# ChrisTho23/DrakeGPT

Measured on AMD Instinct MI355X. Metric: training tokens/sec (fwd+bwd+AdamW), higher is better.
Workload: dtype bf16; 1 GPU; TransformerLM_scaled: V=80 C=384 T=256 heads=6 layers=6 dropout=0.2; fwd+bwd+AdamW; hipGraph=on; batch_per_gpu=64, global_batch=64, seq_len=256, parallelism=dp1, dp_gradient_buckets=1, params=10800464

## Files before the change

drakegpt_amd/_lib.py:

```python
from __future__ import annotations

import ctypes as C
import os

import torch

_HERE = os.path.dirname(os.path.abspath(__file__))
LIB_PATH = os.path.join(_HERE, "lib", "libdrakegpt_hip.so")

DG_F32 = 0
DG_BF16 = 1
DG_FP8_E4M3 = 2
DG_FP8_E5M2 = 3
DG_F32X3 = 4
ABI_VERSION = 21


class GemmNtArgs(C.Structure):
    _fields_ = [
        ("A", C.c_void_p), ("lda", C.c_int64),
        ("B", C.c_void_p), ("ldb", C.c_int64),
        ("C", C.c_void_p), ("ldc", C.c_int64),
        ("M", C.c_int32), ("N", C.c_int32), ("K", C.c_int32),
        ("in_dtype", C.c_int32), ("out_dtype", C.c_int32),
# ... 88 lines not shown
    "dg_gemm_nt_colsum_rows": [C.POINTER(GemmNtArgs)],
    "dg_gemm_nt_sign_bits_bytes": [_i, _i],
    "dg_fp8_amax": [_vp, _i, _i64, _vp, _i, _vp, _vp],
    "dg_fp8_quantize": [_vp, _i, _vp, _i, _i64, _vp, _i, _vp, _vp, _vp],
    "dg_fp8_quantize_delayed": [_vp, _i, _vp, _i, _i64, _vp, _vp, _vp, _vp],
    "dg_gemm_tn": [_vp, _i64, _vp, _i64, _vp, _i64, _i64, _i, _i, _i, _i, _i, _vp],
    "dg_gemm_tn_grouped": [C.POINTER(TnProblem), _i, _i, _vp, _i64, _vp],
    "dg_gemm_tn_grouped_workspace_bytes": [C.POINTER(TnProblem), _i],
    "dg_reduce_partials": [_vp, _i64, _i, _vp, _i64, _vp],
    "dg_colsum": [_vp, _i64, _i, _vp, _i64, _i, _i, _i, _vp],
    "dg_dropout_bwd_cast": [_vp, _i, _i64, _vp, _i64, _i, _i, _i, _f, _vp, _u32, _vp, _i64, _vp, _i64, _i, _vp],
    "dg_cast": [_vp, _i, _vp, _i, _i64, _vp],
    "dg_transpose_cast": [_vp, _i64, _vp, _i64, _i, _i, _i, _vp],
    "dg_transpose_cast_batched": [_vp, _i, _i, _i, _i, _vp],
    "dg_transpose_u8_batched": [_vp, _i, _i, _vp],
    "dg_attn_keep_bits_bytes": [_i, _i, _i, _i, _i],
    "dg_attn_fwd": [_vp, _vp, _vp, _i, _i, _i, _i, _f, _f, _vp, _u32, _i, _vp, _i64, _vp],
    "dg_attn_bwd": [_vp, _vp, _vp, _vp, _vp, _vp, _i64, _i, _i, _i, _i, _f, _f, _vp, _u32, _i, _vp, _i64, _vp],
    "dg_attn_fp8_out_supported": [_i, _i, _i, _i, _i],
    "dg_attn_fwd_fp8": [_vp, _vp, _vp, _i, _i, _i, _i, _f, _f, _vp, _u32, _i, _vp, _i64, C.POINTER(AttnFp8Out), _vp],
    "dg_attn_bwd_fp8": [_vp, _vp, _vp, _vp, _vp, _vp, _i64, _i, _i, _i, _i, _f, _f, _vp, _u32, _i, _vp, _i64, C.POINTER(AttnFp8Out), _vp],
    "dg_attn_bwd_workspace_bytes": [_i, _i, _i, _i, _i],
    "dg_attn_decode": [_vp, _vp, _i, _i, _i, _i, _i, _f, _i, _vp],
    "dg_attn_decode_append": [_vp, _vp, _vp, _vp, _i, _i, _i, _i, _f, _i, _vp],
    "dg_embed_window": [_vp, _i64, _vp, _vp, _vp, _vp, _i, _i, _i, _i, _i, _vp],
    "dg_sample_rows": [_vp, _i64, _i, _i, _vp, _vp, _vp, _i64, _vp, _i64, _vp],
    "dg_sample_rows_nucleus": [_vp, _i64, _i, _i, _vp, _vp, _vp, _i64, _vp, _i64, _vp],
    "dg_cross_entropy": [_vp, _i, _i64, _vp, _vp, _vp, _i64, _i, _f, _vp, _i, _i, _vp],
    "dg_cross_entropy_fp8": [_vp, _i64, _vp, _vp, _vp, _i64, _f, _i, _i, _vp, _i64, _vp],
    "dg_cross_entropy_fused": [_vp, _i64, _vp, _vp, _vp, _i64, _i, _f, _i, _i, _vp, _i64, _i, _vp, _vp, _vp, _f, _vp],
# ... 1 lines not shown
    "dg_cross_entropy_fp8_smooth": [_vp, _i64, _vp, _vp, _vp, _i64, _f, _i, _i, _vp, _i64, _f, _vp],
    "dg_cross_entropy_fused_smooth": [_vp, _i64, _vp, _vp, _vp, _i64, _i, _f, _i, _i, _vp, _i64, _i, _vp, _vp, _vp, _f, _f, _f, _vp],
    "dg_reduce_sum": [_vp, _i64, _f, _vp, _vp],
    "dg_softmax_rows": [_vp, _i64, _vp, _i64, _i, _i, _vp],
    "dg_adamw_step": [_vp, _vp, _vp, _vp, _i64, _vp, _vp, _f, _vp, _i, _vp],
    "dg_sumsq_parts": [_i64],
    "dg_sumsq_partials": [_vp, _i64, _vp, _vp],
    "dg_grad_norm_finalize": [_vp, _i, _f, _vp, _vp, _vp],
    "dg_adamw_step_clip": [_vp, _vp, _vp, _vp, _i64, _vp, _vp, _f, _vp, _vp, _i, _vp],
    "dg_adamw_step_sched": [_vp, _vp, _vp, _vp, _i64, _vp, _vp, _f, _vp, _vp, _i64, _vp, _vp, _i, _vp],
    "dg_adamw_step_ema": [_vp, _vp, _vp, _vp, _i64, _vp, _vp, _f, _vp, _vp, _i64, _vp, _vp, _i, _vp, _vp, _vp],
    "dg_swap_f32": [_vp, _vp, _i64, _vp],
    "dg_grad_accumulate": [_vp, _vp, _i64, _vp, _vp, _vp, _vp, _vp],
    "dg_block_chain_supported": [_i, _i],
    "dg_block_chain_fwd": [C.POINTER(BlockChainArgs), _vp],
    "dg_l2_warm": [_vp, _i64, _vp],
    "dg_pack_chain_weights": [_vp, _i64, _vp, _i, _i, _vp],
    "dg_pack_chain_weights_batched": [_vp, _i, _i, _vp],
    "dg_block_chain_bwd_supported": [_i, _i],
    "dg_block_chain_bwd": [C.POINTER(BlockChainBwdArgs), _vp],
}


def _load() -> C.CDLL:
    if not os.path.exists(LIB_PATH):
        raise RuntimeError(
            f"drakegpt_amd: {LIB_PATH} is missing. Build it with `python -m drakegpt_amd.build` "
            "(needs hipcc; cross-compiles for gfx950 without a GPU). There is no CPU fallback.")
    lib = C.CDLL(LIB_PATH)
    for name, argtypes in SIGNATURES.items():
# ... 27 lines not shown
```

drakegpt_amd/csrc/chain.hip:

```cpp
#include "common.h"
#include <stdlib.h>

typedef __attribute__((address_space(1))) const void* gptr_t;
typedef __attribute__((address_space(3))) void* lptr_t;

#define CH_C 384
#define CH_ROWS 64
#define CH_STAGE_B 24576
#define CH_STAGE_A 4096
#define CH_STAGE (CH_STAGE_B + CH_STAGE_A)
#define CH_NST 4
#define CH_ARES (CH_NST * CH_STAGE)
#define CH_KS (CH_C / 32)

struct ChainP {
    const char* o;
    const float* x;
    const char* wproj; const float* bproj;
    float* x1;
    const float* ln2w; const float* ln2b; float* mean2; float* rstd2; bf16_t* h2;
    const char* w1; const float* b1; bf16_t* f; unsigned char* bits;
    const char* w2; const float* b2;
    float* x2; bf16_t* x2b;
    const float* ln1w; const float* ln1b; float* mean1; float* rstd1; bf16_t* h1;
    const char* wqkv; bf16_t* qkv;
    int M, n_blocks;
    float eps;
    const uint32_t* rng; uint32_t site_proj, site_ffn, thr; float inv_keep; int drop;
    int stagger;
    unsigned long long* stamps;
    int dbg;
};

__device__ __forceinline__ void ch_wait_vm(int n) {
    switch (n) {
        case 6: asm volatile("s_waitcnt vmcnt(6)" ::: "memory"); break;
        case 7: asm volatile("s_waitcnt vmcnt(7)" ::: "memory"); break;
        case 12: asm volatile("s_waitcnt vmcnt(12)" ::: "memory"); break;
        case 13: asm volatile("s_waitcnt vmcnt(13)" ::: "memory"); break;
        case 14: asm volatile("s_waitcnt vmcnt(14)" ::: "memory"); break;
        case 8: asm volatile("s_waitcnt vmcnt(8)" ::: "memory"); break;
        case 18: asm volatile("s_waitcnt vmcnt(18)" ::: "memory"); break;
        case 20: asm volatile("s_waitcnt vmcnt(20)" ::: "memory"); break;
        default: asm volatile("s_waitcnt vmcnt(0)" ::: "memory"); break;
    }
// ... 264 lines not shown
        if (HAS_QKV) warm(w3, p.wqkv, 3 * KS);
        asm volatile("s_waitcnt vmcnt(0)" : "+v"(w0), "+v"(w1), "+v"(w2), "+v"(w3) :: "memory");
    }
    auto stamp = [&](int k) {
        if (p.stamps && wave == 0) {
            const unsigned long long t = __builtin_amdgcn_s_memtime();
            if (lane == 0) p.stamps[(int64_t)blockIdx.x * 24 + k] = t;
        }
    };
    u32x4 fa0[2], fb0[6], fa1[2], fb1[6];
    for (int blk = blockIdx.x; blk < p.n_blocks; blk += gridDim.x) {
        const int64_t row0 = (int64_t)blk * CH_ROWS;
        int g = 0;
        if (MODE == 2) {
            float xv[2][3][8];
#pragma unroll
            for (int q = 0; q < 3; ++q)
#pragma unroll
                for (int i = 0; i < 2; ++i) {
                    const float* xp = p.x + row0 * C + mad24(wm * 32 + i * 16 + fr, C, col_l + 32 * q);
                    const f32x4 a = *(const f32x4*)xp, b = *(const f32x4*)(xp + 4);
#pragma unroll
                    for (int e = 0; e < 4; ++e) { xv[i][q][e] = a[e]; xv[i][q][4 + e] = b[e]; }
                }
            layernorm(xv, (float*)(lds + 0 * CH_STAGE + CH_STAGE_B), row0, p.ln1w, p.ln1b, p.mean1, p.rstd1, p.h1);
        }
        __builtin_amdgcn_s_barrier();
        auto pipe_barrier = [&]() {
            __builtin_amdgcn_sched_barrier(0);
            asm volatile("s_waitcnt lgkmcnt(0)" ::: "memory");
            __builtin_amdgcn_s_barrier();
            __builtin_amdgcn_sched_barrier(0);
        };
        auto piece = [&](int nstep, bool ring_a, bool next, bool a_after_barrier, bool drain = false) {
            read_B(fb0, g);
            if (!a_after_barrier) { if (ring_a) read_A_ring(fa0, g); else read_A_res(fa0, 0); }
            for (int t = 0; t < nstep; t += 2) {
                if (drain && t == nstep - 2 && p.dbg != 10) asm volatile("s_waitcnt vmcnt(0)" ::: "memory");
                if (t == 8) asm volatile("s_waitcnt vmcnt(0)" ::: "memory");
// ... 169 lines not shown
        int dev = 0, n = 256;
        if (hipGetDevice(&dev) == hipSuccess) {
            int x = 0;
            if (hipDeviceGetAttribute(&x, hipDeviceAttributeMultiprocessorCount, dev) == hipSuccess && x > 0) n = x;
        }
        return n;
    }();
    return v;
}

extern "C" int dg_block_chain_supported(int M, int C) { return M > 0 && M % CH_ROWS == 0 && C == CH_C; }

static unsigned long long* g_chain_stamps = nullptr;
extern "C" void dg_debug_set_chain_fwd_stamps(void* q) { g_chain_stamps = (unsigned long long*)q; }

extern "C" int dg_block_chain_fwd(const dg_block_chain_args* a, void* stream) {
    if (!a || !dg_block_chain_supported(a->M, a->C)) return DG_ERR_ARG;
    if (a->mode < 0 || a->mode > 4) return DG_ERR_ARG;
    if (a->dropout_p < 0.f || a->dropout_p >= 1.f) return DG_ERR_ARG;
    const int m = a->mode;
    const bool has_proj = m == 0 || m == 1 || m == 3, has_ffn1 = m == 0 || m == 1, has_ffn2 = m == 0 || m == 1 || m == 4;
    const bool has_qkv = m == 0 || m == 2, ln1 = m == 0 || m == 2 || m == 4;
    auto al = [](const void* q) { return q && dg_aligned16(q); };
    if (!al(a->x) && m != 4) return DG_ERR_ARG;
    if (has_proj && (!al(a->o) || !al(a->wproj) || !al(a->bproj) || !al(a->x1) || !al(a->ln2w) || !al(a->ln2b) || !a->mean2 || !a->rstd2 || !al(a->h2)))
        return DG_ERR_ARG;
    if (has_ffn1 && (!al(a->w1) || !al(a->b1) || !a->sign_bits ||
                     a->sign_bits_bytes < (int64_t)((a->M + 127) / 128) * (4 * a->C / 192) * (128 * 192 / 8))) return DG_ERR_ARG;
    if (has_ffn2 && (!al(a->f) || !al(a->x1) || !al(a->w2) || !al(a->b2) || (m == 1 ? !al(a->x2_bf16) : !al(a->x2)))) return DG_ERR_ARG;
    if (ln1 && (!al(a->ln1w) || !al(a->ln1b) || !a->mean1 || !a->rstd1 || !al(a->h1))) return DG_ERR_ARG;
    if (has_qkv && (!al(a->wqkv) || !al(a->qkv))) return DG_ERR_ARG;
    ChainP p;
    p.o = (const char*)a->o; p.x = a->x; p.wproj = (const char*)a->wproj; p.bproj = a->bproj; p.x1 = a->x1;
    p.ln2w = a->ln2w; p.ln2b = a->ln2b; p.mean2 = a->mean2; p.rstd2 = a->rstd2; p.h2 = (bf16_t*)a->h2;
    p.w1 = (const char*)a->w1; p.b1 = a->b1; p.f = (bf16_t*)a->f; p.bits = a->sign_bits;
    p.w2 = (const char*)a->w2; p.b2 = a->b2; p.x2 = a->x2; p.x2b = (bf16_t*)a->x2_bf16;
    p.ln1w = a->ln1w; p.ln1b = a->ln1b; p.mean1 = a->mean1; p.rstd1 = a->rstd1; p.h1 = (bf16_t*)a->h1;
    p.wqkv = (const char*)a->wqkv; p.qkv = (bf16_t*)a->qkv;
    p.M = a->M; p.n_blocks = a->M / CH_ROWS; p.eps = a->eps;
    p.drop = (a->dropout_p > 0.f && a->rng_state) ? 1 : 0;
    p.rng = a->rng_state; p.site_proj = a->site_proj; p.site_ffn = a->site_ffn;
    p.thr = dg_drop_threshold(a->dropout_p); p.inv_keep = 1.f / (1.f - a->dropout_p);
    { static const int dbg = [] { const char* e = getenv("DG_CHAIN_DBG"); return e ? atoi(e) : 0; }(); p.dbg = dbg; }
    p.stamps = g_chain_stamps;
    { static const int st = [] { const char* e = getenv("DG_CHAIN_STAGGER"); return e ? atoi(e) : 0; }(); p.stagger = st; }
    const dim3 grid(p.n_blocks < ch_num_cus() ? p.n_blocks : ch_num_cus()), block(768);
    hipStream_t s = (hipStream_t)stream;
    switch (m) {
        case 0: hipLaunchKernelGGL(block_chain_fwd_kernel<0>, grid, block, 0, s, p); break;
        case 1: hipLaunchKernelGGL(block_chain_fwd_kernel<1>, grid, block, 0, s, p); break;
        case 2: hipLaunchKernelGGL(block_chain_fwd_kernel<2>, grid, block, 0, s, p); break;
        case 3: hipLaunchKernelGGL(block_chain_fwd_kernel<3>, grid, block, 0, s, p); break;
        default: hipLaunchKernelGGL(block_chain_fwd_kernel<4>, grid, block, 0, s, p); break;
    }
    DG_LAUNCH_CHECK();
    return DG_OK;
}
```

drakegpt_amd/csrc/elementwise.hip:

```cpp
#include "common.h"

__global__ void state_advance_kernel(uint32_t* st) { st[2] += 1u; }

extern "C" int dg_state_advance(uint32_t* rng_state, void* stream) {
    if (!rng_state) return DG_ERR_ARG;
    hipLaunchKernelGGL(state_advance_kernel, dim3(1), dim3(1), 0, (hipStream_t)stream, rng_state);
    DG_LAUNCH_CHECK();
    return DG_OK;
}

__global__ void batch_gather_kernel(const int64_t* __restrict__ corpus, int64_t n_corpus,
                                    const int64_t* __restrict__ off, int64_t* __restrict__ x,
                                    int64_t* __restrict__ y, int B, int T) {
    int64_t i = (int64_t)blockIdx.x * blockDim.x + threadIdx.x;
    if (i >= (int64_t)B * T) return;
    int b = (int)(i / T), t = (int)(i % T);
    int64_t o = off[b] + t;
    int64_t o1 = o + 1;
    if (o < 0) o = 0; if (o >= n_corpus) o = n_corpus - 1;
    if (o1 < 0) o1 = 0; if (o1 >= n_corpus) o1 = n_corpus - 1;
    x[i] = corpus[o];
    y[i] = corpus[o1];
}

// ... 302 lines not shown
    const int R = (int)D[4], Cc = (int)D[5];
    const int local = (int)((int64_t)blockIdx.x - D[6]), tiles_x = (int)D[7];
    const int r0 = (local / tiles_x) * 64, c0 = (local % tiles_x) * 64;
    const int tx = threadIdx.x & 63, ty = threadIdx.x >> 6;
    for (int i = ty; i < 64; i += 4) {
        int r = r0 + i, c = c0 + tx;
        tile[i][tx] = (r < R && c < Cc) ? to_f32<TI>(in[(int64_t)r * ldi + c]) : 0.f;
    }
    __syncthreads();
    for (int i = ty; i < 64; i += 4) {
        int c = c0 + i, r = r0 + tx;
        if (c < Cc && r < ldo) out[(int64_t)c * ldo + r] = from_f32<TO>(tile[tx][i]);
    }
}

__global__ __launch_bounds__(256) void transpose_bf16_batched_kernel(const int64_t* __restrict__ desc, int n_desc) {
    constexpr int PITCH = 68;
    __shared__ __attribute__((aligned(16))) unsigned short tile[64 * PITCH];
    int d = 0;
    for (int i = 1; i < n_desc; ++i)
        if ((int64_t)blockIdx.x >= desc[i * 8 + 6]) d = i;
    const int64_t* D = desc + d * 8;
    const unsigned short* in = (const unsigned short*)D[0];
    unsigned short* out = (unsigned short*)D[1];
    const int64_t ldi = D[2], ldo = D[3];
    const int R = (int)D[4], Cc = (int)D[5];
    const int local = (int)((int64_t)blockIdx.x - D[6]), tiles_x = (int)D[7];
    const int r0 = (local / tiles_x) * 64, c0 = (local % tiles_x) * 64;
    const bool vec = ((ldi | ldo) % 8 == 0) && ((((uintptr_t)in) | ((uintptr_t)out)) % 16 == 0);
#pragma unroll
    for (int pass = 0; pass < 2; ++pass) {
        const int pc = threadIdx.x + 256 * pass, row = pc >> 3, ck = pc & 7;
        const int r = r0 + row, c = c0 + 8 * ck;
        u32x4 v = {0u, 0u, 0u, 0u};
        if (r < R) {
            const unsigned short* src = in + (int64_t)r * ldi + c;
            if (vec && c + 8 <= Cc) v = *(const u32x4*)src;
            else {
                unsigned short e[8];
#pragma unroll
                for (int j = 0; j < 8; ++j) e[j] = (c + j < Cc) ? src[j] : (unsigned short)0;
                v = (u32x4){e[0] | ((uint32_t)e[1] << 16), e[2] | ((uint32_t)e[3] << 16), e[4] | ((uint32_t)e[5] << 16), e[6] | ((uint32_t)e[7] << 16)};
            }
// ... 8 lines not shown
        const int pc = threadIdx.x + 256 * pass, oc = (pc & 7) + 8 * (pc >> 6), rk = (pc >> 3) & 7;
        const int c = c0 + oc, r = r0 + 8 * rk;
        if (c >= Cc || r >= ldo) continue;
        unsigned short e[8];
#pragma unroll
        for (int j = 0; j < 8; ++j) e[j] = tile[(8 * rk + j) * PITCH + oc];
        unsigned short* dstp = out + (int64_t)c * ldo + r;
        if (vec && r + 8 <= ldo)
            *(u32x4*)dstp = (u32x4){e[0] | ((uint32_t)e[1] << 16), e[2] | ((uint32_t)e[3] << 16), e[4] | ((uint32_t)e[5] << 16), e[6] | ((uint32_t)e[7] << 16)};
        else {
#pragma unroll
            for (int j = 0; j < 8; ++j)
                if (r + j < ldo) dstp[j] = e[j];
        }
    }
}

__global__ __launch_bounds__(256) void transpose_u8_batched_kernel(const int64_t* __restrict__ desc, int n_desc) {
    constexpr int PITCH = 144;
    __shared__ __attribute__((aligned(16))) unsigned char ta[128 * PITCH], tb[128 * PITCH];
    int d = 0;
    for (int i = 1; i < n_desc; ++i)
        if ((int64_t)blockIdx.x >= desc[i * 8 + 6]) d = i;
    const int64_t* D = desc + d * 8;
    const unsigned char* in = (const unsigned char*)D[0];
    unsigned char* out = (unsigned char*)D[1];
    const int64_t ldi = D[2], ldo = D[3];
    const int R = (int)D[4], Cc = (int)D[5];
    const int local = (int)((int64_t)blockIdx.x - D[6]), tiles_x = (int)D[7];
    const int r0 = (local / tiles_x) * 128, c0 = (local % tiles_x) * 128;
// ... 650 lines not shown
```

drakegpt_amd/engine.py:

```python
from __future__ import annotations

import contextlib
from typing import Dict, List, Optional, Tuple

import torch

from . import checkpoint as CK
from . import ops
from . import schedules as SCH
from . import sublayers as S
from .model import TransformerLM
from .optim import check_accum_steps, check_max_grad_norm

Tensor = torch.Tensor
ALIGN = 64


def _round(n: int, a: int = ALIGN) -> int:
    return (n + a - 1) // a * a


class _Layout:
    def __init__(self):
        self.entries: Dict[str, Tuple[int, Tuple[int, ...]]] = {}
# ... 182 lines not shown
        self.bf16_logits = self.act == torch.bfloat16 and 4096 < V_ <= 53248 and logits != "fp32" if logits != "bf16" else True
        if self.bf16_logits and (self.act != torch.bfloat16 or not (4096 < V_ <= 53248)):
            raise ValueError("bf16 logits need the bf16 / fp8 precision and a vocabulary of 4097 .. 53248 (the whole-row kernel)")
        g = S.granule(self.act)
        if self.C % g or (self.NH * self.H) % g:
            raise ValueError(f"embedding_dim must be a multiple of {g} for {self.act}")
        self.S = S.n_splits_for(self.M)
        self.G = S.n_partials_for(self.M)
        self.grouped_dw = self.act == torch.bfloat16 and self.M % 64 == 0
        self.last_block_act = _os.environ.get("DG_LAST_BLOCK_ACT", "1") != "0"
        self.fp8_head = False
        self.fp8_dw = self.fp8 and (_os.environ.get("DG_FP8_DW", "1") != "0" if fp8_dw is None else bool(fp8_dw))
        self.chain_full = (_os.environ.get("DG_CHAIN", "1") != "0" and not self.fp8 and self.NH * self.H == self.C and self.last_block_act
                           and ops.block_chain_supported(self.M, self.C, self.act))
        self.chain_warm = _os.environ.get("DG_CHAIN_WARM", "0") == "1"
        self.chain_bwd = (_os.environ.get("DG_CHAIN_BWD", "0") == "1" and self.chain_full and self.stream_dtype == torch.bfloat16
                          and ops.block_chain_bwd_supported(self.M, self.C, self.act))
        self.chain_ln = (_os.environ.get("DG_CHAIN_LN", "0") == "1" and not self.fp8 and self.NH * self.H == self.C
                         and ops.block_chain_supported(self.M, self.C, self.act))
        self._build_layout()
        self.dp_buckets = self._choose_buckets(self._dp_buckets_arg)
        if self.dp_buckets > 1:
            self.chain_bwd = False
        self._alloc_and_adopt()
        if self.fp8_head and self.z_loss > 0.0:
            raise ValueError("z_loss > 0 cannot be combined with the fp8 loss head (precision 'fp8' at a large vocabulary): its "
                             "e5m2 gradient scale rests on |dlogits| <= 1 / M; label_smoothing can")
        self.hyper = torch.tensor([lr, betas[0], betas[1], eps, weight_decay], dtype=torch.float32, device=self.dev)
        self.hyper_host = [float(lr), float(betas[0]), float(betas[1]), float(eps), float(weight_decay)]
        self.lr_table = None if self.lr_table_host is None else self.lr_table_host.to(self.dev)
# ... 262 lines not shown
            wt_off += _round(wt_sizes[key])
        if self.fp8:
            self.seg_f = torch.tensor(seg_f, dtype=torch.int64, device=dev)
            self.seg_b = torch.tensor(seg_b, dtype=torch.int64, device=dev)
            self.w_amax = torch.zeros(len(seg_f) * ops.FP8_AMAX_PARTS, dtype=torch.float32, device=dev)

    def refresh_shadows(self):
        if self.shadow is not None:
            ops.cast(self.flat[:self.layA.size], torch.bfloat16, out=self.shadow[:self.layA.size])
        self._refresh_transposes()

    def _refresh_transposes(self):
        from_shadow = self.shadow is not None
        if getattr(self, "_tr_table", None) is None:
            pairs = [(self.weights.fwd(W) if from_shadow else W, Wt) for W, Wt in self._mats if W.data_ptr() not in self.weights.bwd_stale]
            self._tr_table = ops.make_transpose_table(pairs, self.dev) if pairs else ()
        if self._tr_table:
            ops.transpose_cast_batched(*self._tr_table, self.act, in_dtype=torch.bfloat16 if from_shadow else torch.float32)
        if self._pack_pairs:
            if getattr(self, "_pack_table", None) is None:
                self._pack_table = ops.make_pack_table(self._pack_pairs + self._packT_pairs, self.dev)
            ops.pack_chain_weights_batched(*self._pack_table)
        if self.fp8:
            n = self.seg_f.shape[0]
            ops.fp8_quantize(self.shadow[self.offA:self.offA + self.layA.size], S.E4M3, seg=self.seg_f, n_seg=n, out=self.shadow8,
                             scale_inv=self.wscale_f, amax=self.w_amax)
            if self.fp8_wt8:
                if getattr(self, "_u8_table", None) is None:
                    self._u8_table = ops.make_transpose_u8_table(self._u8_pairs, self.dev)
                ops.transpose_u8_batched(*self._u8_table)
            else:
                ops.fp8_quantize(self.wt_flat, S.E4M3, seg=self.seg_b, n_seg=n, out=self.wt8_flat, scale_inv=self.wscale_b, amax=self.w_amax,
                                 reuse_amax=True)

    def _layer_params(self, l: int):
        pv = self.param_view
        return dict(ln1w=pv(f"{l}.ln1w"), ln1b=pv(f"{l}.ln1b"), wqkv=pv(f"{l}.wqkv"), wproj=pv(f"{l}.wproj"),
                    bproj=pv(f"{l}.bproj"), ln2w=pv(f"{l}.ln2w"), ln2b=pv(f"{l}.ln2b"), w1=pv(f"{l}.w1"), b1=pv(f"{l}.b1"),
                    w2=pv(f"{l}.w2"), b2=pv(f"{l}.b2"))

    def _forward(self, run: S.Run, x_idx: Tensor, y_idx: Optional[Tensor], want_grad: bool, gather: bool = False):
        B, T = x_idx.shape
        M = B * T
        p = self.p_drop
        onehot = self.onehot if (want_grad and self.onehot is not None and M == self.M) else None
        if gather:
            h = ops.batch_embed_fwd(self.corpus, self.off_block, self.state, self.off_ctl, x_idx, y_idx, self.param_view("tok"),
                                    self.param_view("pos"), onehot=onehot).view(M, self.C)
        else:
            h = ops.embed_fwd(x_idx, self.param_view("tok"), self.param_view("pos"), onehot=onehot).view(M, self.C)
        if self.chain_full and ops.block_chain_supported(M, self.C, self.act):
            h, saved = self._blocks_chain(run, h, B, T, want_grad)
            return self._head(run, h, y_idx, want_grad, saved, M)
        saved = []
        pre = None
        for l in range(self.L):
            P = self._layer_params(l)
            nxt = [] if self.chain_ln else None
            h, sa = S.attn_fwd(run, h, P["ln1w"], P["ln1b"], P["wqkv"], P["wproj"], P["bproj"], True, B, T, self.NH, self.H, p, p, l,
                               pre=pre, fuse_ln=(P["ln2w"], P["ln2b"]) if self.chain_ln else None, nxt=nxt)
            pre = nxt[0] if nxt else None
            last = l == self.L - 1
            nxt = [] if (self.chain_ln and not last) else None
            Pn = self._layer_params(l + 1) if nxt is not None else None
            h, sf = S.ffn_fwd(run, h, P["ln2w"], P["ln2b"], P["w1"], P["b1"], P["w2"], P["b2"], True, p, l,
                              out_dtype=self.act if (last and self.last_block_act) else torch.float32,
                              pre=pre, fuse_ln=(Pn["ln1w"], Pn["ln1b"]) if nxt is not None else None, nxt=nxt)
            pre = nxt[0] if nxt else None
            if want_grad:
                saved.append((sa, sf))
        return self._head(run, h, y_idx, want_grad, saved, M)

    def _blocks_chain(self, run: S.Run, h: Tensor, B: int, T: int, want_grad: bool):
        M, C = h.shape
        p = run.p(self.p_drop)
        pk = self.weights.pack
        saved = []
        P = self._layer_params(0)
        r = ops.block_chain_fwd(2, M, C, x=h, ln1w=P["ln1w"], ln1b=P["ln1b"], wqkv=pk(P["wqkv"]))
        x, h1, m1, r1, qkv = h, r["h1"], r["mean1"], r["rstd1"], r["qkv"]
        for l in range(self.L):
            o, lse = ops.attn_fwd(qkv, B, T, self.NH, self.H, self.H ** -0.5, p, run.rng, S.site_attn(l), keep=want_grad)
            last = l == self.L - 1
            if self.chain_warm:
                lo = self.layA.entries[f"{l}.wproj"][0]
                hi = self.layA.entries[f"{l + 1}.wproj"][0] if not last else self.layA.entries["lm.w"][0]
                ops.l2_warm(self.wpack_flat[lo:hi])
            kw = dict(o=o, x=x, wproj=pk(P["wproj"]), bproj=P["bproj"], ln2w=P["ln2w"], ln2b=P["ln2b"], w1=pk(P["w1"]), b1=P["b1"],
                      w2=pk(P["w2"]), b2=P["b2"], dropout_p=p, rng_state=run.rng, site_proj=S.site_proj(l), site_ffn=S.site_ffn(l))
            if last:
                r = ops.block_chain_fwd(1, M, C, **kw)
            else:
                Pn = self._layer_params(l + 1)
                r = ops.block_chain_fwd(0, M, C, ln1w=Pn["ln1w"], ln1b=Pn["ln1b"], wqkv=pk(Pn["wqkv"]), **kw)
# ... 833 lines not shown
```

drakegpt_amd/ops.py:

```python
from __future__ import annotations

import ctypes as C
import math
from typing import Optional

import torch

from . import _lib
from ._lib import DG_BF16, DG_F32, DG_F32X3, DG_FP8_E4M3, DG_FP8_E5M2, GemmNtArgs, check, lib

Tensor = torch.Tensor

_DT = {torch.float32: DG_F32, torch.bfloat16: DG_BF16, torch.float8_e4m3fn: DG_FP8_E4M3, torch.float8_e5m2: DG_FP8_E5M2}
FP8_DTYPES = (torch.float8_e4m3fn, torch.float8_e5m2)
FP8_AMAX_PARTS = 256
ATTN_FP8_HIST = 3 * 64 * 32


def dt_code(dtype: torch.dtype) -> int:
    try:
        return _DT[dtype]
    except KeyError:
        raise TypeError(f"drakegpt_amd: unsupported dtype {dtype} (float32 / bfloat16 / OCP float8 only)") from None

# ... 476 lines not shown
        rows.append([W.data_ptr(), Wt.data_ptr(), _ld(W), ldo, R, Cc, first, tiles_x])
        first += tiles_x * tiles_y
    return torch.tensor(rows, dtype=torch.int64, device=device), len(rows), first


def transpose_u8_batched(table: Tensor, n_desc: int, total_tiles: int) -> None:
    _chk(table, "table", torch.int64)
    check(lib.dg_transpose_u8_batched(_p(table), n_desc, total_tiles, _stream()), "dg_transpose_u8_batched")


def transpose_cast_batched(table: Tensor, n_desc: int, total_tiles: int, dtype: torch.dtype, in_dtype: torch.dtype = torch.float32) -> None:
    _chk(table, "table", torch.int64)
    check(lib.dg_transpose_cast_batched(_p(table), n_desc, total_tiles, dt_code(in_dtype), dt_code(dtype), _stream()), "dg_transpose_cast_batched")


def attn_fp8_out_supported(B: int, T: int, NH: int, H: int, dtype: torch.dtype) -> bool:
    return bool(lib.dg_attn_fp8_out_supported(B, T, NH, H, dt_code(dtype)))


def new_attn_fp8_history(amax: Tensor) -> Tensor:
    return amax.detach().float().reshape(1).expand(ATTN_FP8_HIST).contiguous()


def _attn_fp8_arg(fp8_out, shape, fmt: torch.dtype, dev, only8: bool = False):
    from ._lib import AttnFp8Out
    hist3, step_state = fp8_out
    _chk(hist3, "hist3", torch.float32)
    if hist3.numel() != ATTN_FP8_HIST:
        raise RuntimeError("attention fp8 history must hold ATTN_FP8_HIST floats (ops.new_attn_fp8_history)")
    q8 = torch.empty(shape, dtype=fmt, device=dev)
# ... 484 lines not shown
        N, K = W.shape
        if N % 384 or K % 32:
            raise RuntimeError("pack_chain_weights: N % 384 == 0 and K % 32 == 0 required")
        rows.append([W.data_ptr(), Pk.data_ptr(), N, K, first, _ld(W)])
        first += (N // 384) * (K // 32)
    return torch.tensor(rows, dtype=torch.int64, device=device), len(rows), first


def pack_chain_weights_batched(table: Tensor, n_desc: int, total_stages: int) -> None:
    _chk(table, "table", torch.int64)
    check(lib.dg_pack_chain_weights_batched(_p(table), n_desc, total_stages, _stream()), "dg_pack_chain_weights_batched")


def block_chain_fwd(mode: int, M: int, Cd: int, *, o: Optional[Tensor] = None, x: Optional[Tensor] = None, wproj=None, bproj=None, ln2w=None, ln2b=None,
                    w1=None, b1=None, w2=None, b2=None, ln1w=None, ln1b=None, wqkv=None, f: Optional[Tensor] = None, x1: Optional[Tensor] = None,
                    dropout_p: float = 0.0, rng_state: Optional[Tensor] = None, site_proj: int = 0, site_ffn: int = 0, eps: float = 1e-5) -> dict:
    from ._lib import BlockChainArgs
    dev = next(t for t in (x, o, f) if t is not None).device
    a = BlockChainArgs()
    a.mode, a.M, a.C, a.eps = mode, M, Cd, eps
    out = {}
    has_proj, has_ffn1, has_ffn2 = mode in (0, 1, 3), mode in (0, 1), mode in (0, 1, 4)
    has_qkv, ln1 = mode in (0, 2), mode in (0, 2, 4)

    def new(name, shape, dtype):
        t = out[name] = torch.empty(shape, dtype=dtype, device=dev)
        return t.data_ptr()

    def inp(t, name, dtype, n=None):
        _chk(t, name, dtype)
        if n is not None and t.numel() != n:
            raise RuntimeError(f"block_chain_fwd: {name} must hold {n} values, got {t.numel()}")
# ... 19 lines not shown
        a.w2, a.b2 = inp(w2, "w2", bf, 4 * Cd * Cd), inp(b2, "b2", f32, Cd)
        if mode == 1:
            a.x2_bf16 = new("x2", (M, Cd), bf)
        else:
            a.x2 = new("x2", (M, Cd), f32)
    if ln1:
        a.ln1w, a.ln1b = inp(ln1w, "ln1w", f32, Cd), inp(ln1b, "ln1b", f32, Cd)
        a.mean1, a.rstd1 = new("mean1", (M,), f32), new("rstd1", (M,), f32)
        a.h1 = new("h1", (M, Cd), bf)
    if has_qkv:
        a.wqkv = inp(wqkv, "wqkv", bf, 3 * Cd * Cd)
        a.qkv = new("qkv", (M, 3 * Cd), bf)
    a.dropout_p = float(dropout_p)
    a.rng_state = _p(rng_state) if dropout_p > 0.0 else None
    a.site_proj, a.site_ffn = site_proj, site_ffn
    check(lib.dg_block_chain_fwd(C.byref(a), _stream()), "dg_block_chain_fwd")
    return out


def block_chain_bwd_supported(M: int, C: int, dtype: torch.dtype) -> bool:
    return dtype == torch.bfloat16 and bool(lib.dg_block_chain_bwd_supported(int(M), int(C)))


def block_chain_bwd(mode: int, M: int, Cd: int, *, part_stride: int, dqkv=None, wqkvT=None, x=None, mean1=None, rstd1=None, ln1w=None, dresid1=None,
                    dln1w_part=None, dln1b_part=None, gbias1_part=None, g_in=None, w2T=None, bits=None, db1_part=None, w1T=None, x1=None,
                    mean2=None, rstd2=None, ln2w=None, dresid2=None, dln2w_part=None, dln2b_part=None, gbias2_part=None, wprojT=None,
                    dropout_p: float = 0.0, rng_state: Optional[Tensor] = None, site_ffn_below: int = 0, site_proj: int = 0) -> dict:
    from ._lib import BlockChainBwdArgs
    a = BlockChainBwdArgs()
    a.mode, a.M, a.C = mode, M, Cd
# ... 47 lines not shown
```

include/drakegpt_hip.h:

```cpp
#ifndef DRAKEGPT_HIP_H
#define DRAKEGPT_HIP_H

#include <stdint.h>

#ifdef __cplusplus
extern "C" {
#endif

#define DG_F32 0
#define DG_BF16 1
#define DG_FP8_E4M3 2
#define DG_FP8_E5M2 3
#define DG_F32X3 4

#define DG_OK 0
#define DG_ERR_ARG (-1)
#define DG_ERR_ALIGN (-2)
#define DG_ERR_DTYPE (-3)

#define DG_ABI_VERSION 21

int dg_version(void);
const char* dg_error_string(int code);

// ... 96 lines not shown

int dg_colsum(const void* A, int64_t lda, int dtype, float* part, int64_t part_stride,
              int n_partials, int M, int N, void* stream);

int dg_dropout_bwd_cast(const void* dy, int dy_dtype , int64_t lddy, void* g, int64_t ldg, int dtype,
                        int M, int N, float p, const uint32_t* rng_state, uint32_t site,
                        const float* relu_mask, int64_t ldmask,
                        float* colsum_part, int64_t part_stride, int n_partials, void* stream);

int dg_cast(const void* in, int in_dtype, void* out, int out_dtype, int64_t n, void* stream);
int dg_transpose_cast(const float* in, int64_t ldi, void* out, int64_t ldo, int dtype,
                      int R, int Cc, void* stream);

int dg_transpose_cast_batched(const int64_t* desc, int n_desc, int total_tiles, int in_dtype, int out_dtype, void* stream);
int dg_transpose_u8_batched(const int64_t* desc, int n_desc, int total_tiles, void* stream);

int64_t dg_attn_keep_bits_bytes(int B, int T, int NH, int H, int dtype);
int dg_attn_fwd(const void* qkv, void* out, float* lse, int B, int T, int NH, int H,
                float scale, float dropout_p, const uint32_t* rng_state, uint32_t site,
                int dtype, void* keep_bits, int64_t keep_bits_bytes, void* stream);
int64_t dg_attn_bwd_workspace_bytes(int B, int T, int NH, int H, int dtype);
int dg_attn_bwd(const void* qkv, const void* out, const void* dout, const float* lse,
                void* dqkv, void* workspace, int64_t workspace_bytes, int B, int T, int NH, int H,
                float scale, float dropout_p, const uint32_t* rng_state, uint32_t site,
                int dtype, const void* keep_bits, int64_t keep_bits_bytes, void* stream);

#define DG_ATTN_FP8_HIST (3 * 64 * 32)
typedef struct dg_attn_fp8_out {
    void* q8; float* hist3; const uint32_t* step_state; float* scale_inv; int only8;
} dg_attn_fp8_out;
// ... 68 lines not shown

typedef struct dg_block_chain_args {
    int32_t mode, M, C;
    float eps;
    const void* o; const float* x;
    const void* wproj; const float* bproj; float* x1;
    const float* ln2w; const float* ln2b; float* mean2; float* rstd2; void* h2;
    const void* w1; const float* b1; void* f; uint8_t* sign_bits; int64_t sign_bits_bytes;
    const void* w2; const float* b2; float* x2; void* x2_bf16;
    const float* ln1w; const float* ln1b; float* mean1; float* rstd1; void* h1;
    const void* wqkv; void* qkv;
    float dropout_p; const uint32_t* rng_state; uint32_t site_proj, site_ffn;
} dg_block_chain_args;
int dg_block_chain_supported(int M, int C);
int dg_block_chain_fwd(const dg_block_chain_args* args, void* stream);
int dg_l2_warm(const void* p, int64_t bytes, void* stream);
int dg_pack_chain_weights(const void* w, int64_t ld, void* packed, int N, int K, void* stream);
int dg_pack_chain_weights_batched(const int64_t* desc, int n_desc, int total_stages, void* stream);

typedef struct dg_block_chain_bwd_args {
    int32_t mode, M, C, reserved;
    const void* dqkv; const void* wqkvT; const float* x; const float* mean1; const float* rstd1; const float* ln1w;
    const void* dresid1; void* dx1; void* g1;
    float* dln1w_part; float* dln1b_part; float* gbias1_part;
    const void* g_in;
    const void* w2T; const uint8_t* sign_bits; int64_t sign_bits_bytes; void* df; float* db1_part;
    const void* w1T; const float* x1; const float* mean2; const float* rstd2; const float* ln2w;
    const void* dresid2; void* dx2; void* g2;
    float* dln2w_part; float* dln2b_part; float* gbias2_part;
    const void* wprojT; void* dout;
// ... 11 lines not shown
```

Before: 7.164 million tokens/s.

## Fuse batch embedding into chain kernel and merge weight transpose with packing

The batch gather, token and position embedding, and one-hot write now run inside the first mode-2 block-chain kernel, which also writes the residual x. This removes a separate embedding launch and the round trip of x through memory. A new batched kernel produces the transposed backward copy and the packed chain layout from one read of each bf16 shadow weight, replacing separate transpose and pack launches. The cost is extra register and load work in the chain kernel's prologue and more specialised layout code.

```diff
diff --git a/drakegpt_amd/_lib.py b/drakegpt_amd/_lib.py
--- a/drakegpt_amd/_lib.py
+++ b/drakegpt_amd/_lib.py
@@ -126,6 +126,7 @@
     "dg_transpose_cast": [_vp, _i64, _vp, _i64, _i, _i, _i, _vp],
     "dg_transpose_cast_batched": [_vp, _i, _i, _i, _i, _vp],
     "dg_transpose_u8_batched": [_vp, _i, _i, _vp],
+    "dg_refresh_weight_copies_batched": [_vp, _i, _i, _vp],
     "dg_attn_keep_bits_bytes": [_i, _i, _i, _i, _i],
     "dg_attn_fwd": [_vp, _vp, _vp, _i, _i, _i, _i, _f, _f, _vp, _u32, _i, _vp, _i64, _vp],
     "dg_attn_bwd": [_vp, _vp, _vp, _vp, _vp, _vp, _i64, _i, _i, _i, _i, _f, _f, _vp, _u32, _i, _vp, _i64, _vp],
@@ -157,6 +158,7 @@
     "dg_grad_accumulate": [_vp, _vp, _i64, _vp, _vp, _vp, _vp, _vp],
     "dg_block_chain_supported": [_i, _i],
     "dg_block_chain_fwd": [C.POINTER(BlockChainArgs), _vp],
+    "dg_block_chain_fwd_embed": [C.POINTER(BlockChainArgs), _vp, _i64, _vp, _vp, _vp, _vp, _vp, _vp, _vp, _i, _i, _i, _vp, _i64, _vp],
     "dg_l2_warm": [_vp, _i64, _vp],
     "dg_pack_chain_weights": [_vp, _i64, _vp, _i, _i, _vp],
     "dg_pack_chain_weights_batched": [_vp, _i, _i, _vp],
diff --git a/drakegpt_amd/csrc/chain.hip b/drakegpt_amd/csrc/chain.hip
--- a/drakegpt_amd/csrc/chain.hip
+++ b/drakegpt_amd/csrc/chain.hip
@@ -12,6 +12,13 @@
 #define CH_NST 4
 #define CH_ARES (CH_NST * CH_STAGE)
 #define CH_KS (CH_C / 32)
+
+struct ChainEmbed {
+    const float* tok; const float* pos; float* x_out;
+    const int64_t* corpus; int64_t n_corpus; const int64_t* offsets; const uint32_t* step_state; const uint32_t* ctl;
+    int64_t* x_ids; int64_t* y_ids; bf16_t* onehot; int64_t ld_onehot;
+    int B, T, V;
+};
 
 struct ChainP {
     const char* o;
@@ -29,6 +36,7 @@
     const uint32_t* rng; uint32_t site_proj, site_ffn, thr; float inv_keep; int drop;
     int stagger;
     unsigned long long* stamps;
+    ChainEmbed emb;
     int dbg;
 };
 
@@ -323,15 +331,57 @@
         int g = 0;
         if (MODE == 2) {
             float xv[2][3][8];
-#pragma unroll
-            for (int q = 0; q < 3; ++q)
+            if (p.emb.tok) {
+                const ChainEmbed& E = p.emb;
+                uint32_t orow = 0;
+                if (E.ctl) {
+                    const uint32_t n_rows = E.ctl[1];
+                    orow = E.step_state[2] - E.ctl[0];
+                    if (orow >= n_rows) orow = n_rows ? n_rows - 1 : 0;
+                }
+                const int64_t* off = E.offsets + (int64_t)orow * E.B;
 #pragma unroll
                 for (int i = 0; i < 2; ++i) {
-                    const float* xp = p.x + row0 * C + mad24(wm * 32 + i * 16 + fr, C, col_l + 32 * q);
-                    const f32x4 a = *(const f32x4*)xp, b = *(const f32x4*)(xp + 4);
-#pragma unroll
-                    for (int e = 0; e < 4; ++e) { xv[i][q][e] = a[e]; xv[i][q][4 + e] = b[e]; }
-                }
+                    const int rl = wm * 32 + i * 16 + fr;
+                    const uint32_t m = (uint32_t)row0 + (uint32_t)rl, bq = m / (uint32_t)E.T;
+                    const int t = (int)(m - bq * (uint32_t)E.T);
+                    int64_t o = off[bq] + t, o1 = o + 1;
+                    if (o < 0) o = 0; if (o >= E.n_corpus) o = E.n_corpus - 1;
+                    if (o1 < 0) o1 = 0; if (o1 >= E.n_corpus) o1 = E.n_corpus - 1;
+                    int64_t v = E.corpus[o];
+                    if (wn == 0 && fg == 0) { E.x_ids[m] = v; E.y_ids[m] = E.corpus[o1]; }
+                    v = v < 0 ? 0 : (v >= E.V ? E.V - 1 : v);
+                    if (E.onehot)
+                        for (int j = wn * 4 + fg; (int64_t)j * 8 < E.ld_onehot; j += 16) {
+                            bf16x8 oh;
+#pragma unroll
+                            for (int e = 0; e < 8; ++e) oh[e] = (bf16_t)((int64_t)(j * 8 + e) == v ? 1.f : 0.f);
+                            *(bf16x8*)(E.onehot + (int64_t)m * E.ld_onehot + j * 8) = oh;
+                        }
+                    const float* tp = E.tok + v * C + col_l;
+                    const float* pp = E.pos + mad24(t, C, col_l);
+                    float* xo = E.x_out + row0 * C + mad24(rl, C, col_l);
+#pragma unroll
+                    for (int q = 0; q < 3; ++q) {
+                        const f32x4 a = *(const f32x4*)(tp + 32 * q) + *(const f32x4*)(pp + 32 * q);
+                        const f32x4 b = *(const f32x4*)(tp + 32 * q + 4) + *(const f32x4*)(pp + 32 * q + 4);
+                        *(f32x4*)(xo + 32 * q) = a;
+                        *(f32x4*)(xo + 32 * q + 4) = b;
+#pragma unroll
+                        for (int e = 0; e < 4; ++e) { xv[i][q][e] = a[e]; xv[i][q][4 + e] = b[e]; }
+                    }
+                }
+            } else {
+#pragma unroll
+                for (int q = 0; q < 3; ++q)
+#pragma unroll
+                    for (int i = 0; i < 2; ++i) {
+                        const float* xp = p.x + row0 * C + mad24(wm * 32 + i * 16 + fr, C, col_l + 32 * q);
+                        const f32x4 a = *(const f32x4*)xp, b = *(const f32x4*)(xp + 4);
+#pragma unroll
+                        for (int e = 0; e < 4; ++e) { xv[i][q][e] = a[e]; xv[i][q][4 + e] = b[e]; }
+                    }
+            }
             layernorm(xv, (float*)(lds + 0 * CH_STAGE + CH_STAGE_B), row0, p.ln1w, p.ln1b, p.mean1, p.rstd1, p.h1);
         }
         __builtin_amdgcn_s_barrier();
@@ -531,7 +581,7 @@
 static unsigned long long* g_chain_stamps = nullptr;
 extern "C" void dg_debug_set_chain_fwd_stamps(void* q) { g_chain_stamps = (unsigned long long*)q; }
 
-extern "C" int dg_block_chain_fwd(const dg_block_chain_args* a, void* stream) {
+static int chain_fwd_launch(const dg_block_chain_args* a, const ChainEmbed& emb, void* stream) {
     if (!a || !dg_block_chain_supported(a->M, a->C)) return DG_ERR_ARG;
     if (a->mode < 0 || a->mode > 4) return DG_ERR_ARG;
     if (a->dropout_p < 0.f || a->dropout_p >= 1.f) return DG_ERR_ARG;
@@ -560,6 +610,7 @@
     p.thr = dg_drop_threshold(a->dropout_p); p.inv_keep = 1.f / (1.f - a->dropout_p);
     { static const int dbg = [] { const char* e = getenv("DG_CHAIN_DBG"); return e ? atoi(e) : 0; }(); p.dbg = dbg; }
     p.stamps = g_chain_stamps;
+    p.emb = emb;
     { static const int st = [] { const char* e = getenv("DG_CHAIN_STAGGER"); return e ? atoi(e) : 0; }(); p.stagger = st; }
     const dim3 grid(p.n_blocks < ch_num_cus() ? p.n_blocks : ch_num_cus()), block(768);
     hipStream_t s = (hipStream_t)stream;
@@ -573,3 +624,15 @@
     DG_LAUNCH_CHECK();
     return DG_OK;
 }
+
+extern "C" int dg_block_chain_fwd(const dg_block_chain_args* a, void* stream) { return chain_fwd_launch(a, ChainEmbed{}, stream); }
+
+extern "C" int dg_block_chain_fwd_embed(const dg_block_chain_args* a, const int64_t* corpus, int64_t n_corpus, const int64_t* offsets,
+                                        const uint32_t* step_state, const uint32_t* ctl, int64_t* x_ids, int64_t* y_ids, const float* tok,
+                                        const float* pos, int B, int T, int V, void* onehot, int64_t ld_onehot, void* stream) {
+    if (!a || a->mode != 2 || !corpus || !offsets || !x_ids || !y_ids || !tok || !pos || B <= 0 || T <= 0 || V <= 0 || n_corpus < 2) return DG_ERR_ARG;
+    if ((int64_t)B * T != a->M || (ctl != nullptr) != (step_state != nullptr) || !dg_aligned16(tok) || !dg_aligned16(pos)) return DG_ERR_ARG;
+    if (onehot && (ld_onehot % 8 || ld_onehot < V || (int64_t)(a->C / 4) * 8 < ld_onehot || !dg_aligned16(onehot))) return DG_ERR_ARG;
+    ChainEmbed e{tok, pos, (float*)a->x, corpus, n_corpus, offsets, step_state, ctl, x_ids, y_ids, (bf16_t*)onehot, ld_onehot, B, T, V};
+    return chain_fwd_launch(a, e, stream);
+}
diff --git a/drakegpt_amd/csrc/elementwise.hip b/drakegpt_amd/csrc/elementwise.hip
--- a/drakegpt_amd/csrc/elementwise.hip
+++ b/drakegpt_amd/csrc/elementwise.hip
@@ -340,19 +340,10 @@
     }
 }
 
-__global__ __launch_bounds__(256) void transpose_bf16_batched_kernel(const int64_t* __restrict__ desc, int n_desc) {
-    constexpr int PITCH = 68;
-    __shared__ __attribute__((aligned(16))) unsigned short tile[64 * PITCH];
-    int d = 0;
-    for (int i = 1; i < n_desc; ++i)
-        if ((int64_t)blockIdx.x >= desc[i * 8 + 6]) d = i;
-    const int64_t* D = desc + d * 8;
-    const unsigned short* in = (const unsigned short*)D[0];
-    unsigned short* out = (unsigned short*)D[1];
-    const int64_t ldi = D[2], ldo = D[3];
-    const int R = (int)D[4], Cc = (int)D[5];
-    const int local = (int)((int64_t)blockIdx.x - D[6]), tiles_x = (int)D[7];
-    const int r0 = (local / tiles_x) * 64, c0 = (local % tiles_x) * 64;
+constexpr int TR_PITCH = 68;
+__device__ __forceinline__ void transpose_bf16_tile(const unsigned short* __restrict__ in, unsigned short* __restrict__ out, int64_t ldi, int64_t ldo,
+                                                    int R, int Cc, int r0, int c0, unsigned short* tile) {
+    constexpr int PITCH = TR_PITCH;
     const bool vec = ((ldi | ldo) % 8 == 0) && ((((uintptr_t)in) | ((uintptr_t)out)) % 16 == 0);
 #pragma unroll
     for (int pass = 0; pass < 2; ++pass) {
@@ -391,6 +382,64 @@
                 if (r + j < ldo) dstp[j] = e[j];
         }
     }
+}
+
+__global__ __launch_bounds__(256) void transpose_bf16_batched_kernel(const int64_t* __restrict__ desc, int n_desc) {
+    __shared__ __attribute__((aligned(16))) unsigned short tile[64 * TR_PITCH];
+    int d = 0;
+    for (int i = 1; i < n_desc; ++i)
+        if ((int64_t)blockIdx.x >= desc[i * 8 + 6]) d = i;
+    const int64_t* D = desc + d * 8;
+    const int local = (int)((int64_t)blockIdx.x - D[6]), tiles_x = (int)D[7];
+    transpose_bf16_tile((const unsigned short*)D[0], (unsigned short*)D[1], D[2], D[3], (int)D[4], (int)D[5], (local / tiles_x) * 64, (local % tiles_x) * 64, tile);
+}
+
+__global__ __launch_bounds__(256) void refresh_weight_copies_kernel(const int64_t* __restrict__ desc, int n_desc) {
+    constexpr int PITCH = TR_PITCH;
+    __shared__ __attribute__((aligned(16))) unsigned short tile[128 * PITCH];
+    int d = 0;
+    for (int i = 1; i < n_desc; ++i)
+        if ((int64_t)blockIdx.x >= desc[i * 8 + 7]) d = i;
+    const int64_t* D = desc + d * 8;
+    const unsigned short* in = (const unsigned short*)D[0];
+    unsigned short* out = (unsigned short*)D[1];
+    unsigned short* pk = (unsigned short*)D[2];
+    const int64_t ldi = D[3], ldo = D[4];
+    const int K = (int)D[6];
+    const int local = (int)((int64_t)blockIdx.x - D[7]);
+    if (!pk) {
+        const int tiles_x = (K + 63) >> 6;
+        transpose_bf16_tile(in, out, ldi, ldo, (int)D[5], K, (local / tiles_x) * 64, (local % tiles_x) * 64, tile);
+        return;
+    }
+    const int KT64 = K >> 6, ct = local % KT64, rest = local / KT64, j0 = (rest % 3) * 64, c = rest / 3, c0 = ct * 64;
+#pragma unroll
+    for (int u = 0; u < 4; ++u) {
+        const int pc = threadIdx.x + 256 * u, q = pc & 3, half = (pc >> 2) & 1, ks = (pc >> 3) & 1, jl = pc >> 4, j = j0 + jl;
+        const u32x4 v = *(const u32x4*)(in + (int64_t)(c * 384 + half * 192 + j) * ldi + c0 + ks * 32 + q * 8);
+        const int64_t k = (int64_t)c * (K >> 5) + ct * 2 + ks;
+        *(u32x4*)(pk + (k * 1536 + j * 8 + ((half * 4 + q) ^ (j & 7))) * 8) = v;
+        uint2* dst = (uint2*)(tile + (half * 64 + jl) * PITCH + ks * 32 + q * 8);
+        dst[0] = make_uint2(v[0], v[1]);
+        dst[1] = make_uint2(v[2], v[3]);
+    }
+    __syncthreads();
+#pragma unroll
+    for (int u = 0; u < 4; ++u) {
+        const int pc = threadIdx.x + 256 * u, oc = (pc & 7) + 8 * ((pc >> 6) & 7), rk = (pc >> 3) & 7, half = pc >> 9;
+        unsigned short e[8];
+#pragma unroll
+        for (int j = 0; j < 8; ++j) e[j] = tile[(half * 64 + 8 * rk + j) * PITCH + oc];
+        *(u32x4*)(out + (int64_t)(c0 + oc) * ldo + c * 384 + half * 192 + j0 + 8 * rk) =
+            (u32x4){e[0] | ((uint32_t)e[1] << 16), e[2] | ((uint32_t)e[3] << 16), e[4] | ((uint32_t)e[5] << 16), e[6] | ((uint32_t)e[7] << 16)};
+    }
+}
+
+extern "C" int dg_refresh_weight_copies_batched(const int64_t* desc, int n_desc, int total_tiles, void* stream) {
+    if (!desc || n_desc <= 0 || total_tiles <= 0) return DG_ERR_ARG;
+    hipLaunchKernelGGL(refresh_weight_copies_kernel, dim3(total_tiles), dim3(256), 0, (hipStream_t)stream, desc, n_desc);
+    DG_LAUNCH_CHECK();
+    return DG_OK;
 }
 
 __global__ __launch_bounds__(256) void transpose_u8_batched_kernel(const int64_t* __restrict__ desc, int n_desc) {
diff --git a/drakegpt_amd/engine.py b/drakegpt_amd/engine.py
--- a/drakegpt_amd/engine.py
+++ b/drakegpt_amd/engine.py
@@ -220,6 +220,7 @@
         self.chain_full = (_os.environ.get("DG_CHAIN", "1") != "0" and not self.fp8 and self.NH * self.H == self.C and self.last_block_act
                            and ops.block_chain_supported(self.M, self.C, self.act))
         self.chain_warm = _os.environ.get("DG_CHAIN_WARM", "0") == "1"
+        self.embed_in_chain = self.chain_full and _os.environ.get("DG_EMBED_IN_CHAIN", "1") != "0"
         self.chain_bwd = (_os.environ.get("DG_CHAIN_BWD", "0") == "1" and self.chain_full and self.stream_dtype == torch.bfloat16
                           and ops.block_chain_bwd_supported(self.M, self.C, self.act))
         self.chain_ln = (_os.environ.get("DG_CHAIN_LN", "0") == "1" and not self.fp8 and self.NH * self.H == self.C
@@ -512,12 +513,22 @@
         from_shadow = self.shadow is not None
         if getattr(self, "_tr_table", None) is None:
             pairs = [(self.weights.fwd(W) if from_shadow else W, Wt) for W, Wt in self._mats if W.data_ptr() not in self.weights.bwd_stale]
+            packs = self._pack_pairs + self._packT_pairs
+            packed_of = {src.data_ptr(): pk for src, pk in self._pack_pairs}
+            both = {src.data_ptr() for src, Wt in pairs if src.data_ptr() in packed_of and ops.weight_copies_fusable(src, Wt)}
+            self._copies_table = ()
+            if both and from_shadow and self.act == torch.bfloat16 and _os_env("DG_WEIGHT_COPIES", "1") != "0":
+                self._copies_table = ops.make_weight_copies_table(
+                    [(src, Wt, packed_of[src.data_ptr()] if src.data_ptr() in both else None) for src, Wt in pairs], self.dev)
+                pairs = []
+                packs = [(src, pk) for src, pk in packs if src.data_ptr() not in both]
             self._tr_table = ops.make_transpose_table(pairs, self.dev) if pairs else ()
+            self._pack_table = ops.make_pack_table(packs, self.dev) if packs else ()
+        if self._copies_table:
+            ops.refresh_weight_copies_batched(*self._copies_table)
         if self._tr_table:
             ops.transpose_cast_batched(*self._tr_table, self.act, in_dtype=torch.bfloat16 if from_shadow else torch.float32)
-        if self._pack_pairs:
-            if getattr(self, "_pack_table", None) is None:
-                self._pack_table = ops.make_pack_table(self._pack_pairs + self._packT_pairs, self.dev)
+        if self._pack_table:
             ops.pack_chain_weights_batched(*self._pack_table)
         if self.fp8:
             n = self.seg_f.shape[0]
@@ -542,12 +553,16 @@
         M = B * T
         p = self.p_drop
         onehot = self.onehot if (want_grad and self.onehot is not None and M == self.M) else None
-        if gather:
+        chain = self.chain_full and ops.block_chain_supported(M, self.C, self.act)
+        if gather and chain and self.embed_in_chain:
+            h = dict(corpus=self.corpus, offsets=self.off_block, step_state=self.state, ctl=self.off_ctl, x_ids=x_idx, y_ids=y_idx,
+                     tok=self.param_view("tok"), pos=self.param_view("pos"), onehot=onehot)
+        elif gather:
             h = ops.batch_embed_fwd(self.corpus, self.off_block, self.state, self.off_ctl, x_idx, y_idx, self.param_view("tok"),
                                     self.param_view("pos"), onehot=onehot).view(M, self.C)
         else:
             h = ops.embed_fwd(x_idx, self.param_view("tok"), self.param_view("pos"), onehot=onehot).view(M, self.C)
-        if self.chain_full and ops.block_chain_supported(M, self.C, self.act):
+        if chain:
             h, saved = self._blocks_chain(run, h, B, T, want_grad)
             return self._head(run, h, y_idx, want_grad, saved, M)
         saved = []
@@ -570,12 +585,16 @@
         return self._head(run, h, y_idx, want_grad, saved, M)
 
     def _blocks_chain(self, run: S.Run, h: Tensor, B: int, T: int, want_grad: bool):
-        M, C = h.shape
+        M, C = (B * T, self.C) if isinstance(h, dict) else h.shape
         p = run.p(self.p_drop)
         pk = self.weights.pack
         saved = []
         P = self._layer_params(0)
-        r = ops.block_chain_fwd(2, M, C, x=h, ln1w=P["ln1w"], ln1b=P["ln1b"], wqkv=pk(P["wqkv"]))
+        if isinstance(h, dict):
+            r = ops.block_chain_fwd(2, M, C, embed=h, ln1w=P["ln1w"], ln1b=P["ln1b"], wqkv=pk(P["wqkv"]))
+            h = r["x"]
+        else:
+            r = ops.block_chain_fwd(2, M, C, x=h, ln1w=P["ln1w"], ln1b=P["ln1b"], wqkv=pk(P["wqkv"]))
         x, h1, m1, r1, qkv = h, r["h1"], r["mean1"], r["rstd1"], r["qkv"]
         for l in range(self.L):
             o, lse = ops.attn_fwd(qkv, B, T, self.NH, self.H, self.H ** -0.5, p, run.rng, S.site_attn(l), keep=want_grad)
diff --git a/drakegpt_amd/ops.py b/drakegpt_amd/ops.py
--- a/drakegpt_amd/ops.py
+++ b/drakegpt_amd/ops.py
@@ -514,6 +514,33 @@
     check(lib.dg_transpose_cast_batched(_p(table), n_desc, total_tiles, dt_code(in_dtype), dt_code(dtype), _stream()), "dg_transpose_cast_batched")
 
 
+def make_weight_copies_table(triples, device) -> tuple:
+    rows, first = [], 0
+    for W, Wt, Pk in triples:
+        N, K = W.shape
+        ldo = Wt.shape[1]
+        if Pk is None:
+            tiles = ((K + 63) // 64) * ((ldo + 63) // 64)
+        else:
+            if N % 384 or K % 64 or _ld(W) % 8 or ldo != N or any(t.data_ptr() % 16 for t in (W, Wt, Pk)):
+                raise RuntimeError("refresh_weight_copies: N % 384 == 0, K % 64 == 0, 16-byte aligned rows and ldo == N required")
+            tiles = (N // 384) * 3 * (K // 64)
+        rows.append([W.data_ptr(), Wt.data_ptr(), 0 if Pk is None else Pk.data_ptr(), _ld(W), ldo, N, K, first])
+        first += tiles
+    return torch.tensor(rows, dtype=torch.int64, device=device), len(rows), first
+
+
+def weight_copies_fusable(W: Tensor, Wt: Tensor) -> bool:
+    N, K = W.shape
+    return (W.dtype == torch.bfloat16 and Wt.dtype == torch.bfloat16 and N % 384 == 0 and K % 64 == 0 and _ld(W) % 8 == 0
+            and Wt.shape[1] == N and W.data_ptr() % 16 == 0 and Wt.data_ptr() % 16 == 0)
+
+
+def refresh_weight_copies_batched(table: Tensor, n_desc: int, total_tiles: int) -> None:
+    _chk(table, "table", torch.int64)
+    check(lib.dg_refresh_weight_copies_batched(_p(table), n_desc, total_tiles, _stream()), "dg_refresh_weight_copies_batched")
+
+
 def attn_fp8_out_supported(B: int, T: int, NH: int, H: int, dtype: torch.dtype) -> bool:
     return bool(lib.dg_attn_fp8_out_supported(B, T, NH, H, dt_code(dtype)))
 
@@ -1028,8 +1055,13 @@
 
 def block_chain_fwd(mode: int, M: int, Cd: int, *, o: Optional[Tensor] = None, x: Optional[Tensor] = None, wproj=None, bproj=None, ln2w=None, ln2b=None,
                     w1=None, b1=None, w2=None, b2=None, ln1w=None, ln1b=None, wqkv=None, f: Optional[Tensor] = None, x1: Optional[Tensor] = None,
-                    dropout_p: float = 0.0, rng_state: Optional[Tensor] = None, site_proj: int = 0, site_ffn: int = 0, eps: float = 1e-5) -> dict:
+                    dropout_p: float = 0.0, rng_state: Optional[Tensor] = None, site_proj: int = 0, site_ffn: int = 0, eps: float = 1e-5,
+                    embed: Optional[dict] = None) -> dict:
     from ._lib import BlockChainArgs
+    if embed is not None:
+        if mode != 2 or x is not None:
+            raise ValueError("block_chain_fwd: embed= belongs to mode 2 and replaces x")
+        x = torch.empty((M, Cd), dtype=torch.float32, device=embed["tok"].device)
     dev = next(t for t in (x, o, f) if t is not None).device
     a = BlockChainArgs()
     a.mode, a.M, a.C, a.eps = mode, M, Cd, eps
@@ -1079,6 +1111,26 @@
     a.dropout_p = float(dropout_p)
     a.rng_state = _p(rng_state) if dropout_p > 0.0 else None
     a.site_proj, a.site_ffn = site_proj, site_ffn
+    if embed is not None:
+        e = embed
+        for name, dt in (("corpus", torch.int64), ("offsets", torch.int64), ("x_ids", torch.int64), ("y_ids", torch.int64),
+                         ("tok", f32), ("pos", f32)):
+            _chk(e[name], name, dt)
+        B, T = e["x_ids"].shape
+        onehot, ctl, st = e.get("onehot"), e.get("ctl"), e.get("step_state")
+        if B * T != M or e["y_ids"].shape != e["x_ids"].shape or e["offsets"].dim() != 2 or e["offsets"].shape[1] != B:
+            raise ValueError("block_chain_fwd: x_ids / y_ids must be [B, T] with B * T == M and offsets [n_rows, B]")
+        if (ctl is None) != (st is None):
+            raise ValueError("block_chain_fwd: ctl and step_state go together")
+        if e["tok"].shape[1] != Cd or e["pos"].shape[1] != Cd or T > e["pos"].shape[0]:
+            raise IndexError("block_chain_fwd: tok / pos must be [V, C] / [>= T, C]")
+        if onehot is not None:
+            _chk(onehot, "onehot", bf, contiguous=False)
+        check(lib.dg_block_chain_fwd_embed(C.byref(a), _p(e["corpus"]), e["corpus"].numel(), _p(e["offsets"]), _p(st), _p(ctl), _p(e["x_ids"]),
+                                           _p(e["y_ids"]), _p(e["tok"]), _p(e["pos"]), B, T, e["tok"].shape[0], _p(onehot),
+                                           _ld(onehot) if onehot is not None else 0, _stream()), "dg_block_chain_fwd_embed")
+        out["x"] = x
+        return out
     check(lib.dg_block_chain_fwd(C.byref(a), _stream()), "dg_block_chain_fwd")
     return out
 
diff --git a/include/drakegpt_hip.h b/include/drakegpt_hip.h
--- a/include/drakegpt_hip.h
+++ b/include/drakegpt_hip.h
@@ -134,6 +134,7 @@
 
 int dg_transpose_cast_batched(const int64_t* desc, int n_desc, int total_tiles, int in_dtype, int out_dtype, void* stream);
 int dg_transpose_u8_batched(const int64_t* desc, int n_desc, int total_tiles, void* stream);
+int dg_refresh_weight_copies_batched(const int64_t* desc, int n_desc, int total_tiles, void* stream);
 
 int64_t dg_attn_keep_bits_bytes(int B, int T, int NH, int H, int dtype);
 int dg_attn_fwd(const void* qkv, void* out, float* lse, int B, int T, int NH, int H,
@@ -232,6 +233,9 @@
 } dg_block_chain_args;
 int dg_block_chain_supported(int M, int C);
 int dg_block_chain_fwd(const dg_block_chain_args* args, void* stream);
+int dg_block_chain_fwd_embed(const dg_block_chain_args* args, const int64_t* corpus, int64_t n_corpus, const int64_t* offsets,
+                             const uint32_t* step_state, const uint32_t* ctl, int64_t* x_ids, int64_t* y_ids, const float* tok,
+                             const float* pos, int B, int T, int V, void* onehot, int64_t ld_onehot, void* stream);
 int dg_l2_warm(const void* p, int64_t bytes, void* stream);
 int dg_pack_chain_weights(const void* w, int64_t ld, void* packed, int N, int K, void* stream);
 int dg_pack_chain_weights_batched(const int64_t* desc, int n_desc, int total_stages, void* stream);
```

After: 7.223 million tokens/s, median of 6. About the same (+0.8%).
